# OrientalHorizon/Ray-Tracer-Archive

Measured on NVIDIA B200. Metric: path segments/sec, higher is better.
Workload: dtype f32

## Files before the change

### ray_tracer_archive_b200/csrc/rtb_api.cu

```cuda
#include <cuda_runtime.h>

#include <algorithm>
#include <cmath>
#include <cstdio>
#include <cstring>
#include <string>
#include <vector>

#include <atomic>
#include <memory>
#include <thread>

#include "rtb_device.cuh"
#include "rtb_launch.hpp"
#include "rtb_nccl.hpp"

using namespace rtb;

static thread_local std::string g_err;
static int set_err(int code, const std::string& m) { g_err = m; return code; }
#define CU(call)                                                                                              \
  do {                                                                                                        \
    cudaError_t e_ = (call);                                                                                  \
    if (e_ != cudaSuccess)                                                                                    \
// ... 822 lines not shown
}

static DevPool lane_pool(Lane& L, uint32_t n) {
  DevPool p;
  p.n = n;
  p.n_chunks = (n + RTB_CHUNK - 1) / RTB_CHUNK;
  p.ray = L.ray.p; p.st = L.st.p; p.hit = L.hit.p;
  p.cls = L.cls.p; p.redo[0] = L.redo[0].p; p.redo[1] = L.redo[1].p; p.cursor = L.cursor.p;
  p.c = L.counters.p;
  return p;
}

static int ensure_pix_order(rtb_context* c, uint32_t W, uint32_t H, cudaStream_t st) {
  if (c->pix_w == W && c->pix_h == H && c->pix_order.p) return RTB_OK;
  std::vector<uint32_t> order;
  order.reserve((size_t)W * H);
  for (uint32_t ty = 0; ty < H; ty += 4)
    for (uint32_t tx = 0; tx < W; tx += 8)
      for (uint32_t y = ty; y < std::min(ty + 4, H); ++y)
        for (uint32_t x = tx; x < std::min(tx + 8, W); ++x) order.push_back(y * W + x);
  CU(c->pix_order.upload(order.data(), order.size(), st));
  CU(cudaStreamSynchronize(st));
  c->pix_w = W; c->pix_h = H;
  return RTB_OK;
}

#define RTB_DEFAULT_POOL (1u << 22)

static int check_render_args(rtb_context* c, rtb_scene* s, const rtb_camera* cam, const rtb_params* p, const void* buf) {
  if (!c || !s || !cam || !p || !buf) return set_err(RTB_ERR_INVALID, "NULL argument");
  if (!s->committed) return set_err(RTB_ERR_STATE, "scene not committed (call rtb_scene_commit)");
  if (p->width < 2 || p->height < 2) return set_err(RTB_ERR_INVALID, "image must be at least 2x2 (u = (i+xi)/(W-1), main.rs:752)");
  if (p->max_depth < 1 || p->max_depth > 255) return set_err(RTB_ERR_INVALID, "max_depth must be in [1,255]");
  if (p->spp == 0) return set_err(RTB_ERR_INVALID, "spp must be > 0");
  if ((uint64_t)p->sample_offset + p->spp > (1u << 24)) return set_err(RTB_ERR_INVALID, "sample index exceeds 2^24");
  return RTB_OK;
}

static int render_camera(const rtb_camera& cam, DevCamera& dcam) {
  DevCameraF64 dcam64;
  camera_basis(cam, dcam, dcam64);
  for (int a = 0; a < 3; ++a)
    if (!std::isfinite(dcam.origin[a]) || !std::isfinite(dcam.lmo[a]) || !std::isfinite(dcam.horizontal[a]) || !std::isfinite(dcam.vertical[a]) ||
        !std::isfinite(dcam.u[a]) || !std::isfinite(dcam.v[a]))
      return set_err(RTB_ERR_INVALID, "degenerate camera (non-finite basis: lookfrom == lookat, vup along the view direction, or non-finite arguments)");
  return RTB_OK;
}

static uint32_t extend_opt(const rtb_scene* s) {
  static const char* env_opt = getenv("RTB_OPT");
  return env_opt ? (uint32_t)atoi(env_opt)
         : s->lc.mode == EXTEND_WQ ? ((24u << RTB_OPT_PARK_SHIFT) | (2u << 16))
         : s->lc.mode == EXTEND_DYNAMIC ? (14u << RTB_OPT_PARK_SHIFT)
                                        : (s->lc.all_staged ? 0u : 2u );
}

static int default_lanes() {
  static const int env_lanes = getenv("RTB_LANES") ? atoi(getenv("RTB_LANES")) : 0;
  const int want_lanes = env_lanes > 0 ? env_lanes : 4;
  return std::max(1, std::min(want_lanes, RTB_MAX_LANES));
}

int rtb_render_device(rtb_context* c, rtb_scene* s, const rtb_camera* cam, const rtb_params* p, void* d_accum,
                      void* stream, rtb_stats* stats) {
  int rc = check_render_args(c, s, cam, p, d_accum);
  if (rc) return rc;
  CU(cudaSetDevice(c->device));
  cudaStream_t st = (cudaStream_t)stream;
  const uint64_t npix = (uint64_t)p->width * p->height;
  const bool count = (p->flags & RTB_RENDER_COUNT) != 0, time_ext = (p->flags & RTB_RENDER_TIME_EXTEND) != 0;
  int n_lanes = (count || time_ext) ? 1 : default_lanes();
  if ((uint32_t)n_lanes > p->spp) n_lanes = (int)p->spp;
  uint32_t pool_total = p->pool_paths ? p->pool_paths : RTB_DEFAULT_POOL;
  rc = ensure_pix_order(c, p->width, p->height, st);
  if (rc) return rc;
  DevCamera dcam;
  rc = render_camera(*cam, dcam);
  if (rc) return rc;

  struct LaneRun { DevPool pool; DevParams prm; unsigned long long total; bool active; uint64_t iters, iter_cap; };
  LaneRun run[RTB_MAX_LANES];
  uint32_t first_sample = 0;
  for (int k = 0; k < n_lanes; ++k) {
    Lane& L = c->lanes[k];
    const uint32_t cnt = p->spp / n_lanes + ((uint32_t)k < p->spp % n_lanes ? 1u : 0u);
    LaneRun& R = run[k];
    R.total = npix * cnt;
    uint32_t pool_n = std::max(1024u, pool_total / (uint32_t)n_lanes);
    const uint32_t unit = s->lc.pool_unit;
    if (!p->pool_paths && unit) pool_n = std::max(1u, (pool_n + unit / 2) / unit) * unit;
    if ((unsigned long long)pool_n > R.total) pool_n = (uint32_t)std::max<unsigned long long>(1024ull, R.total);
    rc = ensure_pool(L, pool_n);
    if (rc) return rc;
    R.pool = lane_pool(L, pool_n);
    DevParams& prm = R.prm;
    prm.width = p->width; prm.height = p->height; prm.spp = cnt; prm.sample_offset = p->sample_offset + first_sample;
    prm.max_depth = p->max_depth; prm.rr_start = p->rr_start_depth; prm.seed = p->seed;
    for (int a = 0; a < 3; ++a) prm.bg[a] = p->background[a];
    prm.pix_order = c->pix_order.p;
    prm.inv_npix = 1.0 / (double)npix;
    prm.opt = extend_opt(s);
    prm.inv_wm1 = (float)(1.0 / (double)(p->width - 1));
    prm.inv_hm1 = (float)(1.0 / (double)(p->height - 1));
    prm.accum = (float4*)d_accum;
    first_sample += cnt;
    R.active = true;
    R.iters = 0;
// ... 526 lines not shown
```

### ray_tracer_archive_b200/csrc/rtb_device.cuh

```cuda
#pragma once
#include <cuda_runtime.h>
#include <stdint.h>

#include <cmath>
#include <cstring>

#include "rtb_internal.hpp"

namespace rtb {

#ifdef RTB_CHECKED
__device__ unsigned int g_rtb_check_fail[8];
enum CheckKind : int { CHK_STACK = 0, CHK_NODE = 1, CHK_PRIM = 2, CHK_SLOT = 3, CHK_QUEUE = 4, CHK_LIST = 5 };
#define RTB_CHECK(kind, cond)                          \
  do {                                                 \
    if (!(cond)) atomicAdd(&g_rtb_check_fail[kind], 1u); \
  } while (0)
#else
#define RTB_CHECK(kind, cond) ((void)0)
#endif

#define RTB_MAX_LIGHTS 8
#define RTB_MAX_MEDIA 8
#define RTB_MAX_CHECKER_DEPTH 8
// ... 505 lines not shown
    }
    const float Sz = rcp_fast(dp.z), Sx = dp.x * Sz, Sy = dp.y * Sz;
    const float Ax = __fsub_rn(A.x, __fmul_rn(Sx, A.z)), Ay = __fsub_rn(A.y, __fmul_rn(Sy, A.z));
    const float Bx = __fsub_rn(B.x, __fmul_rn(Sx, B.z)), By = __fsub_rn(B.y, __fmul_rn(Sy, B.z));
    const float Cx = __fsub_rn(C.x, __fmul_rn(Sx, C.z)), Cy = __fsub_rn(C.y, __fmul_rn(Sy, C.z));
    const float U = __fsub_rn(__fmul_rn(Cx, By), __fmul_rn(Cy, Bx));
    const float V = __fsub_rn(__fmul_rn(Ax, Cy), __fmul_rn(Ay, Cx));
    const float W = __fsub_rn(__fmul_rn(Bx, Ay), __fmul_rn(By, Ax));
    const float m = (1.25f * RTB_U22 * amax) * (fabsf(Ax) + fabsf(Ay) + fabsf(Bx) + fabsf(By) + fabsf(Cx) + fabsf(Cy));
    const float mn = fminf(fminf(U, V), W), mx = fmaxf(fmaxf(U, V), W);
    if (mn < -m && mx > m) return HIT_MISS;
    const float det = U + V + W;
    const float idet = rcp_fast(det), za = Sz * A.z, zb = Sz * B.z, zc = Sz * C.z;
    const float zlo = fminf(fminf(za, zb), zc), zhi = fmaxf(fmaxf(za, zb), zc);
    if (!(mn > m || mx < -m)) {
      if (!(zhi >= tmin)) return HIT_MISS;
      t = fmaxf(zlo - RTB_U20 * fabsf(zlo), 0.0f);
      return HIT_AMBIGUOUS;
    }
    t = (U * za + V * zb + W * zc) * idet;
    e = fmaf(RTB_U20, fabsf(t), 4.0f * m * fabsf(idet) * (zhi - zlo));
    if (!(t - e <= tmax_hi)) return HIT_MISS;
    const int st = tmin_status(t, e, tmin);
    if (st == HIT_AMBIGUOUS) t = fmaxf(t - e, 0.0f);
    return st;
  } else {
    const float4 a = __ldg(sc.geom[PT_MOVING] + 2 * idx);
    const float4 b = __ldg(sc.geom[PT_MOVING] + 2 * idx + 1);
    const float3 c = fma3(time, xyz(b), xyz(a));
    return sphere_fast(o, d, c, a.w, tmin, tmax_hi, t, e, coarse);
  }
}
__device__ __forceinline__ void apply_result(Closest& best, float& amb, uint32_t& flags, int st, float t, float e, uint32_t ref,
                                             bool coarse) {
  if (st == HIT_CERTAIN) consider(best, amb, flags, t, e, ref, coarse);
  else if (st == HIT_AMBIGUOUS) undecided(best, amb, t);
}
template <bool COUNT>
__device__ __forceinline__ void intersect_prim(const DevScene& sc, uint32_t type, uint32_t idx, float3 o, float3 d,
                                               float time, float tmin, Closest& best, float& amb, uint32_t& flags, TestCount& n_tests) {
  float t, e;
  bool coarse;
  const int st = prim_test<COUNT>(sc, type, idx, o, d, time, tmin, best.hi, t, e, coarse, n_tests);
  apply_result(best, amb, flags, st, t, e, (type << REF_TYPE_SHIFT) | idx, coarse);
}

__device__ __forceinline__ float q2f(uint32_t word, uint32_t magic, uint32_t sel) {
  return __uint_as_float(__byte_perm(word, magic, sel));
}

#if !defined(__CUDA_ARCH__) && defined(RTB_EMUL_STATS)
inline unsigned long long g_emul_stats[8];
inline float g_emul_tmax0 = INFINITY;
#endif
struct Trav {
  float3 o, d;
  float idx, idy, idz, time;
  uint32_t octinv;
  uint2 grp;
  int sp;
  Closest best;
  float amb;
};
__device__ __forceinline__ uint32_t octant_remap(uint32_t m, uint32_t octinv) {
  if (octinv & 1u) m = ((m & 0x55u) << 1) | ((m & 0xAAu) >> 1);
  if (octinv & 2u) m = ((m & 0x33u) << 2) | ((m & 0xCCu) >> 2);
  if (octinv & 4u) m = ((m & 0x0Fu) << 4) | ((m & 0xF0u) >> 4);
  return m;
}
__shared__ uint8_t s_octmap[8 * 256];
__device__ __forceinline__ bool needs_exact(const Closest& best, float amb) { return amb < INFINITY && amb <= best.hi; }
enum FixKind : uint32_t { FIX_NONE = 0, FIX_RETRACE = 1, FIX_REFINE = 2 };
#define RTB_REDO_REFINE 0x80000000u
__device__ __forceinline__ bool quad_distance_is_coarse(const DevScene& sc, uint32_t idx, float3 o, float3 d) {
  const float4 w0 = __ldg(sc.geom[PT_QUAD] + 3 * idx);
  if (__ldg(&sc.info[PT_QUAD][idx].y) >> 31) return false;
  const float mag_num = fabsf(w0.w) + fabsf(w0.x * o.x) + fabsf(w0.y * o.y) + fabsf(w0.z * o.z);
  const float mag_den = fabsf(w0.x * d.x) + fabsf(w0.y * d.y) + fabsf(w0.z * d.z);
  return 64.0f * fabsf(dot(xyz(w0), d)) < mag_den || 64.0f * fabsf(w0.w - dot(xyz(w0), o)) < mag_num;
}
__device__ __forceinline__ bool tri_distance_is_coarse(const DevScene& sc, uint32_t idx, float3 o, float3 d) {
  const float3 v0 = xyz(__ldg(sc.geom[PT_TRI] + 3 * idx));
  const float3 n = cross(xyz(__ldg(sc.geom[PT_TRI] + 3 * idx + 1)) - v0, xyz(__ldg(sc.geom[PT_TRI] + 3 * idx + 2)) - v0);
  const float3 r = v0 - o;
  const float mag_num = fabsf(n.x * r.x) + fabsf(n.y * r.y) + fabsf(n.z * r.z);
  const float mag_den = fabsf(n.x * d.x) + fabsf(n.y * d.y) + fabsf(n.z * d.z);
  return 64.0f * fabsf(dot(n, d)) < mag_den || 64.0f * fabsf(dot(n, r)) < mag_num;
}
#define FIX_NOMINATED 3u
__device__ __forceinline__ uint32_t fix_kind_cheap(const Trav& tv) {
  if (needs_exact(tv.best, tv.amb)) return FIX_RETRACE;
  if (tv.best.ref == REF_MISS) return FIX_NONE;
  const uint32_t type = tv.best.ref >> REF_TYPE_SHIFT;
  if (type == PT_QUAD || type == PT_TRI)
    return tv.best.hi - tv.best.t > (type == PT_QUAD ? RTB_FLAT_REL_MAX : RTB_TRI_REL_MAX) * tv.best.t ? FIX_NOMINATED : FIX_NONE;
  return (tv.octinv & RTB_TRAV_COARSE) ? FIX_REFINE : FIX_NONE;
}
__device__ __forceinline__ uint32_t resolve_nominated(const DevScene& sc, uint32_t ref, float3 o, float3 d) {
  const uint32_t type = ref >> REF_TYPE_SHIFT, idx = ref & REF_INDEX_MASK;
  const bool coarse = type == PT_QUAD ? quad_distance_is_coarse(sc, idx, o, d) : tri_distance_is_coarse(sc, idx, o, d);
  return coarse ? FIX_REFINE : FIX_NONE;
}
__device__ __forceinline__ uint32_t fix_kind(const DevScene& sc, const Trav& tv) {
  const uint32_t k = fix_kind_cheap(tv);
  return k == FIX_NOMINATED ? resolve_nominated(sc, tv.best.ref, tv.o, tv.d) : k;
}
// ... 122 lines not shown
      const float tnx = fmaf(q2f(i < 4 ? nx0 : nx1, magic, sel), ax, bnx);
      const float tny = fmaf(q2f(i < 4 ? ny0 : ny1, magic, sel), ay, bny);
      const float tnz = fmaf(q2f(i < 4 ? nz0 : nz1, magic, sel), az, bnz);
      const float tfx = fmaf(q2f(i < 4 ? fx0 : fx1, magic, sel), ax, bfx);
      const float tfy = fmaf(q2f(i < 4 ? fy0 : fy1, magic, sel), ay, bfy);
      const float tfz = fmaf(q2f(i < 4 ? fz0 : fz1, magic, sel), az, bfz);
      const float tn = fmaxf(fmaxf(tnx, tny), tnz);
      const float tf = fminf(fminf(tfx, tfy), tfz);
      const uint32_t neg = __float_as_uint(tf - tn) | __float_as_uint(tmax - tn) | __float_as_uint(tf - tmin);
      missmask = __funnelshift_l(neg, missmask, 1);
    }
  }
  const uint32_t hitmask = ~missmask & 0xFFu;
#if !defined(__CUDA_ARCH__) && defined(RTB_EMUL_STATS)
  ++g_emul_stats[0];
  if (!hitmask) ++g_emul_stats[1];
  g_emul_stats[2] += __builtin_popcount(hitmask & imask);
  g_emul_stats[3] += __builtin_popcount(hitmask & ~imask);
  {
    uint32_t np = 0;
    for (uint32_t s = 0; s < 8; ++s)
      if ((hitmask & ~imask) >> s & 1u) np += (((s < 4 ? w1.z : w1.w) >> (8 * (s & 3))) & 0xFFu) >> 5;
    if (np) ++g_emul_stats[np == 1 ? 4 : (np == 2 ? 5 : 6)];
    g_emul_stats[7] += np;
  }
#endif
  uint32_t ih = hitmask & imask;
  if constexpr (OCTMAP) ih = s_octmap[(octinv << 8) | ih];
  else ih = octant_remap(ih, octinv);
  tv.grp = make_uint2(w1.x, (ih << 8) | imask);
  const uint32_t leaf = hitmask & ~imask;
  if (leaf) leaves_fn(leaf, w1.y, w1.z, w1.w);
  return true;
}

template <bool COUNT>
__device__ __forceinline__ void trav_globals(const DevScene& sc, Trav& tv, float tmin, TestCount& n_tests) {
  for (uint32_t k = 0; k < sc.n_global; ++k) {
    const uint32_t ref = sc.global_ref[k];
    if ((sc.global_f64 >> k) & 1u) {
      if (COUNT) ++n_tests.n[PT_SPHERE];
      const float4 s = __ldg(sc.geom[PT_SPHERE] + (ref & REF_INDEX_MASK));
      float t;
      const int st = sphere_roots_f64(tv.o, tv.d, xyz(s), s.w, tmin, t);
      if (st == HIT_CERTAIN) consider(tv.best, tv.amb, tv.octinv, t, RTB_U22 * t, ref, false);
      else if (st == HIT_AMBIGUOUS) tv.amb = 0.0f;
    } else {
      intersect_prim<COUNT>(sc, ref >> REF_TYPE_SHIFT, ref & REF_INDEX_MASK, tv.o, tv.d, tv.time, tmin, tv.best, tv.amb, tv.octinv, n_tests);
    }
  }
  if (sc.tree_empty) tv.grp.y = 0u;
}

template <bool COUNT, bool ALL_STAGED = false, bool PACKED = false, bool OCTMAP = false, bool SPHSTAGE = false>
__device__ __forceinline__ bool trav_step_fast(const DevScene& sc, const uint4* __restrict__ snodes, uint32_t sbase, uint32_t n_snodes,
                                               Trav& tv, uint2* __restrict__ stack, float tmin,
                                               uint32_t& n_nodes_visited, TestCount& n_tests, uint32_t ssph = 0u) {
  return trav_step<COUNT, ALL_STAGED, 1, PACKED, OCTMAP>(sc, snodes, sbase, n_snodes, tv, stack, tmin, n_nodes_visited,
                                      [&](uint32_t leaf, uint32_t w1y, uint32_t w1z, uint32_t w1w) {
                                        expand_leaves(leaf, w1y, w1z, w1w, [&](uint32_t type, uint32_t idx) {
                                          if (SPHSTAGE && type == PT_SPHERE) {
                                            if (COUNT) ++n_tests.n[PT_SPHERE];
                                            RTB_CHECK(CHK_PRIM, idx < sc.n_prims[PT_SPHERE]);
                                            float t, e = 0.0f;
                                            bool coarse = false;
                                            const float4 s = lds_sphere(sc, ssph, idx);
                                            const int st = sphere_fast(tv.o, tv.d, xyz(s), s.w, tmin, tv.best.hi, t, e, coarse);
                                            apply_result(tv.best, tv.amb, tv.octinv, st, t, e, ((uint32_t)PT_SPHERE << REF_TYPE_SHIFT) | idx, coarse);
                                          } else {
                                            intersect_prim<COUNT>(sc, type, idx, tv.o, tv.d, tv.time, tmin, tv.best, tv.amb, tv.octinv, n_tests);
                                          }
                                        });
                                      });
}

template <bool COUNT, bool ALL_STAGED = false>
__device__ __forceinline__ bool trav_step_park(const DevScene& sc, const uint4* __restrict__ snodes, uint32_t sbase, uint32_t n_snodes,
                                               Trav& tv, uint2* __restrict__ stack, float tmin, uint32_t& n_nodes_visited,
                                               uint4* __restrict__ park, bool& parked) {
  return trav_step<COUNT, ALL_STAGED, 1, false>(sc, snodes, sbase, n_snodes, tv, stack, tmin, n_nodes_visited,
                                      [&](uint32_t leaf, uint32_t w1y, uint32_t w1z, uint32_t w1w) {
                                        *park = make_uint4(leaf, w1y, w1z, w1w);
                                        parked = true;
                                      });
}
template <bool COUNT>
__device__ __forceinline__ void drain_parked(const DevScene& sc, Trav& tv, float tmin, const uint4* __restrict__ park, bool parked,
                                             TestCount& n_tests) {
  uint4 pd = make_uint4(0u, 0u, 0u, 0u);
  if (parked) pd = *park;
  const uint32_t mytype = pd.y >> REF_TYPE_SHIFT;
#pragma unroll
  for (uint32_t t = 0; t < PT_COUNT; ++t) {
    const bool mine = parked && mytype == t;
    if (!__any_sync(0xffffffffu, mine)) continue;
    if (mine)
      expand_leaves(pd.x, pd.y, pd.z, pd.w, [&](uint32_t, uint32_t idx) {
        intersect_prim<COUNT>(sc, t, idx, tv.o, tv.d, tv.time, tmin, tv.best, tv.amb, tv.octinv, n_tests);
      });
    __syncwarp();
  }
}

template <bool COUNT, bool ALL_STAGED = false, bool PACKED = false, bool OCTMAP = false, bool SPHSTAGE = false>
__device__ __forceinline__ uint32_t traverse(const DevScene& sc, const uint4* __restrict__ snodes, uint32_t sbase, uint32_t n_snodes,
                                         float3 o, float3 d, float time, float tmin, Closest& best, float& slab_lo_out,
                                         uint32_t& n_nodes_visited, TestCount& n_tests, uint32_t ssph = 0u) {
  Trav tv;
  uint2 stack[RTB_STACK];
  trav_init(tv, o, d, time);
  trav_globals<COUNT>(sc, tv, tmin, n_tests);
  while (trav_step_fast<COUNT, ALL_STAGED, PACKED, OCTMAP, SPHSTAGE>(sc, snodes, sbase, n_snodes, tv, stack, tmin, n_nodes_visited, n_tests, ssph)) {}
  best = tv.best;
  slab_lo_out = slab_lo(tv);
  return fix_kind(sc, tv);
}

__device__ __forceinline__ float refine_hit(const DevScene& sc, uint32_t ref, float3 o, float3 d, float time, float t) {
  if ((ref >> REF_TYPE_SHIFT) >= PT_COUNT) return t;
  const double tc = exact_hit(sc.xtab, ref, o, d, time);
  return tc >= 0.0 ? (float)tc : t;
}

__device__ __forceinline__ Closest traverse_exact(const DevScene& sc, float3 o, float3 d, float time, float t_lo = 0.0f, float t_hi = INFINITY) {
  Trav tv;
  uint2 stack[RTB_STACK];
  trav_init(tv, o, d, time);
  tv.best.hi = fmaf(t_hi, 4.0e-6f, t_hi) + 1.0e-6f;
  const float tmin = fmaxf(fmaf(t_lo, -4.0e-6f, t_lo) - 1.0e-6f, 0.0f);
  double bt = 0.0;
  const ExactTab* tab = sc.xtab;
  auto leaf = [&](uint32_t type, uint32_t idx) {
    const uint32_t ref = (type << REF_TYPE_SHIFT) | idx;
    {
      Closest probe{INFINITY, tv.best.hi, REF_MISS};
      float probe_amb = INFINITY;
      uint32_t probe_flags = 0;
      TestCount none{};
      intersect_prim<false>(sc, type, idx, tv.o, tv.d, tv.time, RTB_TMIN, probe, probe_amb, probe_flags, none);
      if (probe.ref == REF_MISS && !(probe_amb < INFINITY)) return;
    }
    const double tc = exact_hit(tab, ref, tv.o, tv.d, tv.time);
    if (tc < 0.0) return;
    if (tv.best.ref == REF_MISS || tc < bt || (tc == bt && tab_gid(tab, ref) > tab_gid(tab, tv.best.ref))) {
      bt = tc;
      const float tf = (float)tc;
      tv.best.t = tf;
      tv.best.hi = tf * (1.0f + RTB_U22);
      tv.best.ref = ref;
    }
  };
  for (uint32_t k = 0; k < sc.n_global; ++k) leaf(sc.global_ref[k] >> REF_TYPE_SHIFT, sc.global_ref[k] & REF_INDEX_MASK);
  if (sc.tree_empty) tv.grp.y = 0u;
  uint32_t nv = 0;
  while (trav_step<false, false>(sc, nullptr, 0u, 0u, tv, stack, tmin, nv,
                                 [&](uint32_t lf, uint32_t w1y, uint32_t w1z, uint32_t w1w) { expand_leaves(lf, w1y, w1z, w1w, leaf); })) {}
  if (tv.best.ref == REF_MISS) tv.best.t = tv.best.hi = INFINITY;
  return tv.best;
}

__device__ __forceinline__ void intersect_media(const DevScene& sc, float3 o, float3 d, float tmin, Closest& best,
                                                uint32_t pixel, uint32_t sample, uint32_t bounce, uint32_t seed,
                                                bool have_rng) {
  for (uint32_t m = 0; m < sc.n_media; ++m) {
    const DevMedium& md = sc.media[m];
// ... 51 lines not shown
```

### ray_tracer_archive_b200/csrc/rtb_kernels.cu

```cuda
#include <cuda_runtime.h>

#include <algorithm>
#include <cstdlib>
#include <cstring>

#include "rtb_device.cuh"
#include "rtb_launch.hpp"

namespace rtb {

__device__ __forceinline__ uint32_t ray_octant(float3 d) {
  return (d.x < 0.0f ? 1u : 0u) | (d.y < 0.0f ? 2u : 0u) | (d.z < 0.0f ? 4u : 0u);
}

__device__ __forceinline__ void prefetch_l1(const void* p) { asm volatile("prefetch.global.L1 [%0];" ::"l"(p)); }
__device__ __forceinline__ void prefetch_l2(const void* p) { asm volatile("prefetch.global.L2 [%0];" ::"l"(p)); }

__device__ __forceinline__ void red_add_v4(float4* addr, float a, float b, float c, float d) {
  asm volatile("red.global.add.v4.f32 [%0], {%1, %2, %3, %4};" ::"l"(addr), "f"(a), "f"(b), "f"(c), "f"(d) : "memory");
}

__device__ __forceinline__ void deposit(const DevParams& prm, DevCounters* c, uint32_t pixel, float3 L) {
  if (!(isfinite(L.x) && isfinite(L.y) && isfinite(L.z))) {
    atomicAdd(&c->rejected, 1ull);
// ... 123 lines not shown
  for (uint32_t j = 0; j < 8; ++j) {
    const uint32_t b = ((j < 4 ? cw.x : cw.y) >> (8 * (j & 3))) & 0xFFu, cls = b & 7u;
    key[j] = cls == CLS_DEAD ? 64u : ((cls == CLS_NEW ? 0u : cls + 1u) << 3) | ((b >> 3) & 7u);
    rank[j] = key[j] < 64u ? atomicAdd(&cnt[key[j]], 1u) : 0u;
  }
  __syncwarp();
  const uint32_t v0 = cnt[lane], v1 = lane < 16u ? cnt[32u + lane] : 0u;
  uint32_t i0 = v0, i1 = v1;
#pragma unroll
  for (uint32_t d = 1; d < 32; d <<= 1) {
    const uint32_t a = __shfl_up_sync(0xffffffffu, i0, d), b2 = __shfl_up_sync(0xffffffffu, i1, d);
    if (lane >= d) { i0 += a; i1 += b2; }
  }
  const uint32_t t0 = __shfl_sync(0xffffffffu, i0, 31), total = t0 + __shfl_sync(0xffffffffu, i1, 15);
  __syncwarp();
  cnt[lane] = i0 - v0;
  if (lane < 16u) cnt[32u + lane] = t0 + i1 - v1;
  __syncwarp();
#pragma unroll
  for (uint32_t j = 0; j < 8; ++j)
    if (key[j] < 64u) {
      RTB_CHECK(CHK_LIST, cnt[key[j]] + rank[j] < RTB_CHUNK);
      list[cnt[key[j]] + rank[j]] = (uint8_t)(8u * lane + j);
    }
  __syncwarp();
  return total;
}

__device__ __forceinline__ void report_counts(DevCounters* c, uint32_t nv, TestCount nt, uint32_t lane) {
  nv = __reduce_add_sync(0xffffffffu, nv);
  uint32_t tot = 0;
#pragma unroll
  for (uint32_t t = 0; t < PT_COUNT; ++t) {
    nt.n[t] = __reduce_add_sync(0xffffffffu, nt.n[t]);
    tot += nt.n[t];
  }
  if (lane == 0) {
    atomicAdd(&c->nodes_visited, (unsigned long long)nv);
    atomicAdd(&c->prims_tested, (unsigned long long)tot);
    for (uint32_t t = 0; t < PT_COUNT; ++t)
      if (nt.n[t]) atomicAdd(&c->prims_tested_type[t], (unsigned long long)nt.n[t]);
  }
}

#ifndef RTB_EXTEND_MAXREG
#define RTB_EXTEND_MAXREG 80
#endif
#ifndef RTB_EXTEND_DYN_MAXREG
#define RTB_EXTEND_DYN_MAXREG 64
#endif
struct ExtIn { float4 o_time, d_slot, idir_oct, best; };
struct ExtOut { float t; uint32_t ref, slot, redo; float lo, hi; uint32_t _pad[2]; };
#define RTB_EXTEND_WARPS (RTB_EXTEND_THREADS / 32)

template <bool COUNT>
__global__ void __maxnreg__(RTB_EXTEND_DYN_MAXREG)
k_extend(DevScene sc, DevPool pool, DevParams prm, uint32_t n_snodes) {
  extern __shared__ uint4 snodes[];
  __shared__ ExtIn s_in[RTB_EXTEND_WARPS][32];
  __shared__ ExtOut s_out[RTB_EXTEND_WARPS][32];
  __shared__ uint8_t s_list[RTB_EXTEND_WARPS][RTB_CHUNK];
  __shared__ uint4 s_park[RTB_EXTEND_WARPS][32];
  DevCounters* c = pool.c;
  stage_nodes(sc, snodes, n_snodes);
  uint32_t sbase = (uint32_t)__cvta_generic_to_shared(snodes);
  asm volatile("mov.u32 %0, %0;" : "+r"(sbase));
  const uint32_t lane = threadIdx.x & 31u, warp = threadIdx.x >> 5;
  const uint32_t lt_mask = (1u << lane) - 1u;
  const uint32_t park_min = max(1u, (prm.opt >> RTB_OPT_PARK_SHIFT) & RTB_OPT_PARK_MASK);
  uint4* park = &s_park[warp][lane];
  uint32_t parked_mask = 0;
  ExtIn* in = s_in[warp];
  ExtOut* out = s_out[warp];
  uint8_t* list = s_list[warp];
  uint32_t idle = 0xffffffffu;
  uint32_t slot = 0;
  uint32_t in_head = 0, in_count = 0, out_count = 0;
  uint32_t chunk_base = 0, list_pos = 0, list_len = 0;
  bool exhausted = false;
  uint32_t n_rays = 0;
  Trav tv;
  uint2 stack[RTB_STACK];
  uint32_t nv = 0;
  TestCount nt{};
  const uint32_t refill_min = 8u;
  auto flush = [&]() {
    __syncwarp();
    if (lane < out_count) {
      const ExtOut h = out[lane];
      float3 o = f3(0.f, 0.f, 0.f), d = o;
      if (sc.n_media) {
        o = xyz(pool.ray[2 * h.slot]);
        d = xyz(pool.ray[2 * h.slot + 1]);
      }
      finish_ray(sc, pool, prm, h.slot, o, d, Closest{h.t, h.t, h.ref});
      uint32_t redo = h.redo;
      if (redo == FIX_NOMINATED) redo = resolve_nominated(sc, h.ref, xyz(pool.ray[2 * h.slot]), xyz(pool.ray[2 * h.slot + 1]));
      if (redo) queue_fix(pool, h.slot, redo, h.lo, h.hi);
    }
    out_count = 0;
    __syncwarp();
  };

  for (;;) {
    const uint32_t n_idle = __popc(idle);
    if (n_idle >= refill_min || idle == 0xffffffffu) {
// ... 248 lines not shown
      finished = !trav_step<COUNT, false, (int)RTB_WQ_RAYS>(sc, snodes, sbase, n_snodes, tv, &W.stack[0][r], RTB_TMIN, nv,
                                                            [&](uint32_t leaf, uint32_t w1y, uint32_t w1z, uint32_t w1w) {
                                                              W.rec[r] = make_uint4(leaf, w1y, w1z, w1w);
                                                              const uint32_t type = w1y >> REF_TYPE_SHIFT;
                                                              cls = type <= PT_MOVING ? 0u : type - 1u;
                                                              leafed = true;
                                                            });
      RTB_CHECK(CHK_STACK, tv.sp <= (int)RTB_WQ_STACK);
      if (!finished) {
        *reinterpret_cast<uint2*>(&W.trav[r]) = tv.grp;
        W.trav[r].z = (uint32_t)tv.sp;
      }
    }
    const uint32_t done = __ballot_sync(0xffffffffu, finished);
    const uint32_t leafs = __ballot_sync(0xffffffffu, leafed);
    if (done | leafs) {
      const uint32_t bit_lo = r < 32u ? 1u << r : 0u, bit_hi = (r & 32u) ? 1u << (r & 31u) : 0u;
      rdy_lo &= ~__reduce_or_sync(0xffffffffu, finished || leafed ? bit_lo : 0u);
      rdy_hi &= ~__reduce_or_sync(0xffffffffu, finished || leafed ? bit_hi : 0u);
      if (leafs) {
        const uint32_t m0 = __ballot_sync(0xffffffffu, cls == 0u), m1 = __ballot_sync(0xffffffffu, cls == 1u), m2 = leafs & ~(m0 | m1);
        if (leafed) {
          const uint32_t mine = cls == 0u ? m0 : (cls == 1u ? m1 : m2);
          const uint32_t end = cls == 0u ? qh0 + qn0 : (cls == 1u ? qh1 + qn1 : qh2 + qn2);
          W.q[cls][(end + __popc(mine & lt_mask)) & 63u] = (uint8_t)r;
        }
        qn0 += __popc(m0); qn1 += __popc(m1); qn2 += __popc(m2);
      }
      if (done) {
        free_lo |= __reduce_or_sync(0xffffffffu, finished ? bit_lo : 0u);
        free_hi |= __reduce_or_sync(0xffffffffu, finished ? bit_hi : 0u);
        if (out_count + __popc(done) > 32u) flush();
        if (finished) {
          const float4 b = W.best[r];
          Trav tv;
          tv.best = Closest{b.x, b.z, __float_as_uint(b.y)};
          tv.amb = b.w;
          tv.octinv = W.trav[r].w;
          W.out[out_count + __popc(done & lt_mask)] =
              ExtOut{tv.best.t, tv.best.ref, __float_as_uint(W.d_slot[r].w), fix_kind_cheap(tv), slab_lo(tv), tv.best.hi, {0u, 0u}};
        }
        out_count += __popc(done);
      }
    }
    __syncwarp();
  }
  if (lane == 0 && n_rays) atomicAdd(&c->iter_rays, n_rays);
  if (COUNT) report_counts(c, nv, nt, lane);
}

template <bool COUNT, bool ALL_STAGED, bool SORT, bool SPHSTAGE = false>
__global__ void __maxnreg__(RTB_EXTEND_MAXREG)
k_extend_static(DevScene sc, DevPool pool, DevParams prm, uint32_t n_snodes) {
  static_assert(!SPHSTAGE || (ALL_STAGED && !COUNT), "the sphere stage is built for the fully staged production kernel");
  extern __shared__ uint4 snodes[];
  __shared__ uint8_t s_list[RTB_EXTEND_WARPS][RTB_CHUNK];
  __shared__ uint32_t s_cnt[SORT ? RTB_EXTEND_WARPS : 1][64];
  DevCounters* c = pool.c;
  if constexpr (ALL_STAGED) octmap_fill();
  if constexpr (SPHSTAGE) {
    const uint4* sph = reinterpret_cast<const uint4*>(sc.geom[PT_SPHERE]);
    for (uint32_t i = threadIdx.x; i < sc.n_prims[PT_SPHERE]; i += blockDim.x) snodes[5u * n_snodes + i] = __ldg(sph + i);
  }
  stage_nodes(sc, snodes, n_snodes);
  uint32_t sbase = (uint32_t)__cvta_generic_to_shared(snodes);
  asm volatile("mov.u32 %0, %0;" : "+r"(sbase));
  const uint32_t lane = threadIdx.x & 31u, warp = threadIdx.x >> 5;
  uint8_t* list = s_list[warp];
  const uint32_t n_warps = gridDim.x * RTB_EXTEND_WARPS;
  uint32_t n_rays = 0, nv = 0;
  TestCount nt{};
  for (uint32_t chunk = blockIdx.x * RTB_EXTEND_WARPS + warp; chunk < pool.n_chunks; chunk += n_warps) {
    const uint32_t base = chunk * RTB_CHUNK;
    const uint32_t total = SORT ? build_extend_list_sorted(pool, chunk, list, s_cnt[SORT ? warp : 0], lane) : build_extend_list(pool, chunk, list, lane);
    n_rays += total;
    for (uint32_t r = 0; r < total; r += 32) {
      if (r + 32 + lane < total) prefetch_l1(pool.ray + 2 * (size_t)(base + list[r + 32 + lane]));
      if (r + lane < total) {
        const uint32_t slot = base + list[r + lane];
        const float4 ro = pool.ray[2 * slot];
        const float4 rd = pool.ray[2 * slot + 1];
        Closest best;
        float lo;
        const uint32_t fix = traverse<COUNT, ALL_STAGED, ALL_STAGED && !COUNT, ALL_STAGED, SPHSTAGE>(
            sc, snodes, sbase, n_snodes, xyz(ro), xyz(rd), ro.w, RTB_TMIN, best, lo, nv, nt, sbase + n_snodes * 80u);
        finish_ray(sc, pool, prm, slot, xyz(ro), xyz(rd), best);
        if (fix) queue_fix(pool, slot, fix, lo, best.hi);
      }
    }
    __syncwarp();
  }
  if (lane == 0 && n_rays) atomicAdd(&c->iter_rays, n_rays);
  if (COUNT) report_counts(c, nv, nt, lane);
}

struct Surf {
  float3 p, n, outward;
  bool front;
  uint32_t mat, ref;
};

__device__ __forceinline__ Surf surface_at(const DevScene& sc, uint32_t ref, uint32_t minfo, float3 o, float3 d, float time, float t) {
  Surf s;
  s.ref = ref;
  s.p = fma3(t, d, o);
  const uint32_t type = ref >> REF_TYPE_SHIFT, idx = ref & REF_INDEX_MASK;
  if (type == PT_MEDIUM) {
    s.n = s.outward = f3(1.f, 0.f, 0.f);
    s.front = true;
    s.mat = RTB_MINFO_MAT(minfo);
    return s;
  }
  if (type == PT_SPHERE) {
    const float4 g = __ldg(sc.geom[PT_SPHERE] + idx);
    s.outward = rcp_fast(g.w) * (s.p - xyz(g));
  } else if (type == PT_MOVING) {
    const float4 a = __ldg(sc.geom[PT_MOVING] + 2 * idx), b = __ldg(sc.geom[PT_MOVING] + 2 * idx + 1);
    s.outward = rcp_fast(a.w) * (s.p - fma3(time, xyz(b), xyz(a)));
  } else if (type == PT_QUAD) {
    s.outward = xyz(__ldg(sc.geom[PT_QUAD] + 3 * idx));
  } else {
    const float3 v0 = xyz(__ldg(sc.geom[PT_TRI] + 3 * idx));
    const float3 e1 = xyz(__ldg(sc.geom[PT_TRI] + 3 * idx + 1)) - v0, e2 = xyz(__ldg(sc.geom[PT_TRI] + 3 * idx + 2)) - v0;
    s.outward = unit(cross(e1, e2));
  }
  s.mat = RTB_MINFO_MAT(minfo);
  bool ff = dot(d, s.outward) < 0.0f;
  s.n = ff ? s.outward : -s.outward;
  const uint32_t mode = RTB_MINFO_FACE(minfo), base = mode & 7u;
  if (mode >= FACE_Q) {
    float sn, cs;
    if (type == PT_TRI) {
      sn = __ldg(sc.geom[PT_TRI] + 3 * idx).w;
      cs = __ldg(sc.geom[PT_TRI] + 3 * idx + 1).w;
    } else {
      const double* ex = sc.xtab->exact[type] + (size_t)idx * RTB_EXACT_STRIDE;
      sn = (float)ex[4]; cs = (float)ex[5];
    }
// ... 644 lines not shown
  extern __shared__ uint4 sm[];
  const uint32_t n = 2048;
  for (uint32_t i = threadIdx.x; i < n; i += blockDim.x) sm[i] = make_uint4(i, i * 3u, i * 5u, i * 7u);
  __syncthreads();
  uint4 acc = make_uint4(0u, 0u, 0u, 0u);
  const uint32_t base = (uint32_t)__cvta_generic_to_shared(sm);
  uint32_t k = threadIdx.x;
#pragma unroll 8
  for (uint32_t r = 0; r < reps; ++r) {
    uint4 v;
    asm volatile("ld.shared.v4.u32 {%0, %1, %2, %3}, [%4];" : "=r"(v.x), "=r"(v.y), "=r"(v.z), "=r"(v.w) : "r"(base + k * 16u));
    acc.x ^= v.x; acc.y ^= v.y; acc.z ^= v.z; acc.w ^= v.w;
    k = (k + 256u) & (n - 1u);
  }
  if ((acc.x ^ acc.y ^ acc.z ^ acc.w) == 0x12345679u) sink[0] = acc;
}

#ifdef RTB_CHECKED
int read_check_failures(unsigned int* out8) {
  return (int)cudaMemcpyFromSymbol(out8, g_rtb_check_fail, sizeof(unsigned int) * 8);
}
#else
int read_check_failures(unsigned int* out8) {
  for (int i = 0; i < 8; ++i) out8[i] = 0xFFFFFFFFu;
  return 0;
}
#endif

static inline uint32_t cdiv(uint32_t a, uint32_t b) { return (a + b - 1) / b; }

void launch_init_pool(const DevPool& pool, unsigned long long total_paths, cudaStream_t st) {
  k_init_pool<<<cdiv(pool.n_chunks * RTB_CHUNK, 256), 256, 0, st>>>(pool, total_paths);
}
void launch_generate(const LaunchCfg& lc, const DevPool& pool, const DevParams& prm, const DevCamera& cam, cudaStream_t st) {
  k_generate<<<lc.shade_grid, RTB_SHADE_THREADS, 0, st>>>(pool, prm, cam);
}
void launch_fixup(const LaunchCfg& lc, const DevScene& sc, const DevPool& pool, const DevParams& prm, cudaStream_t st) {
  k_fixup<<<lc.fixup_grid, RTB_FIXUP_THREADS, 0, st>>>(sc, pool, prm);
}
void launch_rotate(const DevPool& pool, cudaStream_t st) { k_rotate<<<1, 1, 0, st>>>(pool); }
void launch_extend(const LaunchCfg& lc, const DevScene& sc, const DevPool& pool, const DevParams& prm, bool count,
                   cudaStream_t st) {
  if (lc.mode == EXTEND_WQ) {
    if (count) k_extend_wq<true><<<lc.extend_grid, RTB_EXTEND_THREADS, lc.extend_smem, st>>>(sc, pool, prm, lc.n_snodes);
    else k_extend_wq<false><<<lc.extend_grid, RTB_EXTEND_THREADS, lc.extend_smem, st>>>(sc, pool, prm, lc.n_snodes);
    return;
  }
  if (lc.mode == EXTEND_STATIC) {
    const bool sort = (prm.opt & RTB_OPT_OCTANT_SORT) != 0u;
    if (count) {
      if (sort) k_extend_static<true, false, true><<<lc.extend_grid, RTB_EXTEND_THREADS, lc.extend_smem, st>>>(sc, pool, prm, lc.n_snodes);
      else k_extend_static<true, false, false><<<lc.extend_grid, RTB_EXTEND_THREADS, lc.extend_smem, st>>>(sc, pool, prm, lc.n_snodes);
    } else if (lc.all_staged && lc.sphere_smem) {
      const uint32_t smem = lc.extend_smem + lc.sphere_smem;
      if (sort) k_extend_static<false, true, true, true><<<lc.extend_grid, RTB_EXTEND_THREADS, smem, st>>>(sc, pool, prm, lc.n_snodes);
      else k_extend_static<false, true, false, true><<<lc.extend_grid, RTB_EXTEND_THREADS, smem, st>>>(sc, pool, prm, lc.n_snodes);
    } else if (lc.all_staged) {
      if (sort) k_extend_static<false, true, true><<<lc.extend_grid, RTB_EXTEND_THREADS, lc.extend_smem, st>>>(sc, pool, prm, lc.n_snodes);
      else k_extend_static<false, true, false><<<lc.extend_grid, RTB_EXTEND_THREADS, lc.extend_smem, st>>>(sc, pool, prm, lc.n_snodes);
    } else {
      if (sort) k_extend_static<false, false, true><<<lc.extend_grid, RTB_EXTEND_THREADS, lc.extend_smem, st>>>(sc, pool, prm, lc.n_snodes);
      else k_extend_static<false, false, false><<<lc.extend_grid, RTB_EXTEND_THREADS, lc.extend_smem, st>>>(sc, pool, prm, lc.n_snodes);
    }
    return;
  }
  if (count) k_extend<true><<<lc.extend_grid, RTB_EXTEND_THREADS, lc.extend_smem, st>>>(sc, pool, prm, lc.n_snodes);
  else k_extend<false><<<lc.extend_grid, RTB_EXTEND_THREADS, lc.extend_smem, st>>>(sc, pool, prm, lc.n_snodes);
}
void launch_shade(const LaunchCfg& lc, const DevScene& sc, const DevPool& pool, const DevParams& prm,
                  const DevCamera& cam, uint32_t present, cudaStream_t st) {
  k_shade_terminal<<<lc.shade_grid, RTB_SHADE_THREADS, 0, st>>>(sc, pool, prm, cam);
  if (present & (1u << RTB_MAT_LAMBERTIAN)) k_shade_lambert<<<lc.shade_grid, RTB_SHADE_THREADS, 0, st>>>(sc, pool, prm, cam);
  if (present & ((1u << RTB_MAT_METAL) | (1u << RTB_MAT_DIELECTRIC)))
    k_shade_specular<<<lc.shade_grid, RTB_SHADE_THREADS, 0, st>>>(sc, pool, prm, cam);
  if (present & (1u << RTB_MAT_ISOTROPIC)) k_shade_isotropic<<<lc.shade_grid, RTB_SHADE_THREADS, 0, st>>>(sc, pool, prm, cam);
}
void launch_finalize(const float4* accum, uint8_t* rgb, uint32_t npix, float inv_spp, cudaStream_t st) {
  k_finalize<<<cdiv(npix, 256), 256, 0, st>>>(accum, rgb, npix, inv_spp);
}
void launch_probe_fill(const DevPool& pool, const float* org, const float* dir, const float* time, uint32_t n, cudaStream_t st) {
  k_probe_fill<<<cdiv(pool.n_chunks * RTB_CHUNK, 256), 256, 0, st>>>(pool, org, dir, time, n);
}
void launch_probe_collect(const DevScene& sc, const DevPool& pool, uint32_t n, uint32_t* id_out, float* t_out, cudaStream_t st) {
  k_probe_collect<<<cdiv(n, 256), 256, 0, st>>>(sc, pool, n, id_out, t_out);
}
void launch_kat(const DevScene& sc, const DevCamera& cam, const DevParams& prm, uint32_t op, const uint32_t* in, uint32_t n,
                uint32_t in_stride, uint32_t* out, uint32_t out_stride, cudaStream_t st) {
  k_kat<<<cdiv(n, 128), 128, 0, st>>>(sc, cam, prm, op, in, n, in_stride, out, out_stride);
}
void launch_bw_global(const uint4* p, size_t n_vec, uint32_t reps, uint4* sink, uint32_t grid, cudaStream_t st) {
  k_bw_global<<<grid, 256, 0, st>>>(p, n_vec, reps, sink);
}
void launch_bw_shared(uint32_t reps, uint4* sink, uint32_t grid, cudaStream_t st) {
  k_bw_shared<<<grid, 256, 32768, st>>>(reps, sink);
}
void launch_aov_fill(const DevPool& pool, const DevParams& prm, const DevCamera& cam, unsigned long long first_path,
                     uint32_t n, cudaStream_t st) {
  k_aov_fill<<<cdiv(pool.n_chunks * RTB_CHUNK, 256), 256, 0, st>>>(pool, prm, cam, first_path, n);
}
void launch_aov_collect(const DevScene& sc, const DevPool& pool, const DevParams& prm, float4* aov, uint32_t n,
                        cudaStream_t st) {
  k_aov_collect<<<cdiv(n, RTB_SHADE_THREADS), RTB_SHADE_THREADS, 0, st>>>(sc, pool, prm, aov, n);
}
void launch_primary_rays(const DevCameraF64& cam, uint32_t W, uint32_t H, float* org, float* dir, float* time,
                         cudaStream_t st) {
  k_primary_rays<<<cdiv(W * H, 256), 256, 0, st>>>(cam, W, H, org, dir, time);
}

int configure_launch(LaunchCfg& lc, uint32_t n_nodes, uint32_t max_depth, uint32_t n_spheres, int sm_count) {
  lc.dynamic_fetch = n_nodes > 4096;
  uint32_t budget = (getenv("RTB_STAGE_KB") ? (uint32_t)atoi(getenv("RTB_STAGE_KB")) : (lc.dynamic_fetch ? 6u : 12u)) * 1024u;
  budget = std::min(budget, (lc.dynamic_fetch ? 84u : 104u) * 1024u);
  uint32_t n_s = n_nodes;
  if ((size_t)n_s * 80 > budget) n_s = budget / 80;
  lc.n_snodes = n_s;
  lc.all_staged = n_s == n_nodes && !(getenv("RTB_ALL_STAGED") && atoi(getenv("RTB_ALL_STAGED")) == 0);
  lc.extend_smem = n_s * 80;
  const char* mode = getenv("RTB_EXTEND_MODE");
  lc.mode = lc.dynamic_fetch ? EXTEND_DYNAMIC : EXTEND_STATIC;
  if (mode) lc.mode = !strcmp(mode, "static") ? EXTEND_STATIC : (!strcmp(mode, "wq") ? EXTEND_WQ : EXTEND_DYNAMIC);
  if (lc.mode == EXTEND_WQ && (lc.all_staged || max_depth + 2u > RTB_WQ_STACK))
    lc.mode = lc.dynamic_fetch ? EXTEND_DYNAMIC : EXTEND_STATIC;
  lc.sphere_smem = lc.mode == EXTEND_STATIC && lc.all_staged && n_spheres <= RTB_SPHERE_STAGE_BYTES / 16u ? n_spheres * 16u : 0u;
  cudaError_t e;
  const void* extend_fn = (const void*)k_extend<false>;
  if (lc.mode == EXTEND_WQ) {
    const uint32_t wq_bytes = RTB_EXTEND_WARPS * (uint32_t)sizeof(WqWarp);
    lc.extend_smem += wq_bytes;
    extend_fn = (const void*)k_extend_wq<false>;
    for (const void* fn : {(const void*)k_extend_wq<false>, (const void*)k_extend_wq<true>}) {
      e = cudaFuncSetAttribute(fn, cudaFuncAttributeMaxDynamicSharedMemorySize, (int)(budget + wq_bytes));
      if (e != cudaSuccess) return (int)e;
    }
  }
  e = cudaFuncSetAttribute(k_extend<false>, cudaFuncAttributeMaxDynamicSharedMemorySize, (int)budget);
  if (e != cudaSuccess) return (int)e;
  e = cudaFuncSetAttribute(k_extend<true>, cudaFuncAttributeMaxDynamicSharedMemorySize, (int)budget);
  if (e != cudaSuccess) return (int)e;
  for (const void* fn : {(const void*)k_extend_static<true, false, false>, (const void*)k_extend_static<true, false, true>,
                         (const void*)k_extend_static<false, true, false>, (const void*)k_extend_static<false, true, true>,
                         (const void*)k_extend_static<false, false, false>, (const void*)k_extend_static<false, false, true>}) {
    e = cudaFuncSetAttribute(fn, cudaFuncAttributeMaxDynamicSharedMemorySize, (int)budget);
    if (e != cudaSuccess) return (int)e;
  }
  if (lc.sphere_smem) {
    for (const void* fn : {(const void*)k_extend_static<false, true, false, true>, (const void*)k_extend_static<false, true, true, true>}) {
      e = cudaFuncSetAttribute(fn, cudaFuncAttributeMaxDynamicSharedMemorySize, (int)(budget + RTB_SPHERE_STAGE_BYTES));
      if (e != cudaSuccess) return (int)e;
    }
  }
  int occ = 0;
  e = cudaOccupancyMaxActiveBlocksPerMultiprocessor(&occ, extend_fn, RTB_EXTEND_THREADS, lc.extend_smem + lc.sphere_smem);
  if (e != cudaSuccess) return (int)e;
  if (occ < 1) occ = 1;
  occ = std::min(occ, getenv("RTB_EXTEND_OCC") ? std::max(1, atoi(getenv("RTB_EXTEND_OCC"))) : std::max(1, 512 / RTB_EXTEND_THREADS));
  lc.extend_grid = (uint32_t)(sm_count * occ);
  int occ2 = 0;
  e = cudaOccupancyMaxActiveBlocksPerMultiprocessor(&occ2, k_shade_lambert, RTB_SHADE_THREADS, 0);
  if (e != cudaSuccess) return (int)e;
  if (occ2 < 1) occ2 = 1;
  if (getenv("RTB_SHADE_OCC")) occ2 = std::max(1, std::min(occ2, atoi(getenv("RTB_SHADE_OCC"))));
  lc.shade_grid = (uint32_t)(sm_count * occ2);
  lc.fixup_grid = (uint32_t)std::max(1, sm_count * 2);
  {
    uint32_t a = lc.extend_grid * RTB_EXTEND_WARPS, b = lc.shade_grid * RTB_SHADE_WARPS, x = a, y = b;
    while (y) { const uint32_t t = x % y; x = y; y = t; }
    const uint64_t lcm = (uint64_t)a / x * b;
    lc.pool_unit = lcm * RTB_CHUNK <= (1ull << 23) ? (uint32_t)(lcm * RTB_CHUNK) : b * RTB_CHUNK;
  }
  return 0;
}

}
```

Before: 8490.

## Add persistent ray refill and leaf parking to sphere-staged static extend kernel

```diff
diff --git a/ray_tracer_archive_b200/csrc/rtb_api.cu b/ray_tracer_archive_b200/csrc/rtb_api.cu
--- a/ray_tracer_archive_b200/csrc/rtb_api.cu
+++ b/ray_tracer_archive_b200/csrc/rtb_api.cu
@@ -898,7 +898,7 @@
   return env_opt ? (uint32_t)atoi(env_opt)
          : s->lc.mode == EXTEND_WQ ? ((24u << RTB_OPT_PARK_SHIFT) | (2u << 16))
          : s->lc.mode == EXTEND_DYNAMIC ? (14u << RTB_OPT_PARK_SHIFT)
-                                        : (s->lc.all_staged ? 0u : 2u );
+                                        : (s->lc.all_staged ? (8u << RTB_OPT_PARK_SHIFT) : 2u );
 }
 
 static int default_lanes() {
diff --git a/ray_tracer_archive_b200/csrc/rtb_device.cuh b/ray_tracer_archive_b200/csrc/rtb_device.cuh
--- a/ray_tracer_archive_b200/csrc/rtb_device.cuh
+++ b/ray_tracer_archive_b200/csrc/rtb_device.cuh
@@ -581,6 +581,11 @@
 #if !defined(__CUDA_ARCH__) && defined(RTB_EMUL_STATS)
 inline unsigned long long g_emul_stats[8];
 inline float g_emul_tmax0 = INFINITY;
+inline uint8_t* g_emul_seq = nullptr;
+inline unsigned long long g_emul_seq_n = 0, g_emul_seq_cap = 0;
+inline void emul_seq_push(uint32_t v) {
+  if (g_emul_seq && g_emul_seq_n < g_emul_seq_cap) g_emul_seq[g_emul_seq_n++] = (uint8_t)(v == 255u || v < 254u ? v : 254u);
+}
 #endif
 struct Trav {
   float3 o, d;
@@ -809,26 +814,32 @@
   if (sc.tree_empty) tv.grp.y = 0u;
 }
 
-template <bool COUNT, bool ALL_STAGED = false, bool PACKED = false, bool OCTMAP = false, bool SPHSTAGE = false>
+template <bool COUNT, bool ALL_STAGED = false, bool PACKED = false, bool OCTMAP = false>
 __device__ __forceinline__ bool trav_step_fast(const DevScene& sc, const uint4* __restrict__ snodes, uint32_t sbase, uint32_t n_snodes,
                                                Trav& tv, uint2* __restrict__ stack, float tmin,
-                                               uint32_t& n_nodes_visited, TestCount& n_tests, uint32_t ssph = 0u) {
+                                               uint32_t& n_nodes_visited, TestCount& n_tests) {
   return trav_step<COUNT, ALL_STAGED, 1, PACKED, OCTMAP>(sc, snodes, sbase, n_snodes, tv, stack, tmin, n_nodes_visited,
                                       [&](uint32_t leaf, uint32_t w1y, uint32_t w1z, uint32_t w1w) {
                                         expand_leaves(leaf, w1y, w1z, w1w, [&](uint32_t type, uint32_t idx) {
-                                          if (SPHSTAGE && type == PT_SPHERE) {
-                                            if (COUNT) ++n_tests.n[PT_SPHERE];
-                                            RTB_CHECK(CHK_PRIM, idx < sc.n_prims[PT_SPHERE]);
-                                            float t, e = 0.0f;
-                                            bool coarse = false;
-                                            const float4 s = lds_sphere(sc, ssph, idx);
-                                            const int st = sphere_fast(tv.o, tv.d, xyz(s), s.w, tmin, tv.best.hi, t, e, coarse);
-                                            apply_result(tv.best, tv.amb, tv.octinv, st, t, e, ((uint32_t)PT_SPHERE << REF_TYPE_SHIFT) | idx, coarse);
-                                          } else {
-                                            intersect_prim<COUNT>(sc, type, idx, tv.o, tv.d, tv.time, tmin, tv.best, tv.amb, tv.octinv, n_tests);
-                                          }
+                                          intersect_prim<COUNT>(sc, type, idx, tv.o, tv.d, tv.time, tmin, tv.best, tv.amb, tv.octinv, n_tests);
                                         });
                                       });
+}
+
+template <bool COUNT>
+__device__ __forceinline__ void leaf_test_staged(const DevScene& sc, Trav& tv, float tmin, uint32_t type, uint32_t idx,
+                                                 TestCount& n_tests, uint32_t ssph) {
+  if (type == PT_SPHERE) {
+    if (COUNT) ++n_tests.n[PT_SPHERE];
+    RTB_CHECK(CHK_PRIM, idx < sc.n_prims[PT_SPHERE]);
+    float t, e = 0.0f;
+    bool coarse = false;
+    const float4 s = lds_sphere(sc, ssph, idx);
+    const int st = sphere_fast(tv.o, tv.d, xyz(s), s.w, tmin, tv.best.hi, t, e, coarse);
+    apply_result(tv.best, tv.amb, tv.octinv, st, t, e, ((uint32_t)PT_SPHERE << REF_TYPE_SHIFT) | idx, coarse);
+  } else {
+    intersect_prim<COUNT>(sc, type, idx, tv.o, tv.d, tv.time, tmin, tv.best, tv.amb, tv.octinv, n_tests);
+  }
 }
 
 template <bool COUNT, bool ALL_STAGED = false>
@@ -859,15 +870,24 @@
   }
 }
 
-template <bool COUNT, bool ALL_STAGED = false, bool PACKED = false, bool OCTMAP = false, bool SPHSTAGE = false>
+template <bool COUNT, bool ALL_STAGED = false, bool PACKED = false, bool OCTMAP = false>
 __device__ __forceinline__ uint32_t traverse(const DevScene& sc, const uint4* __restrict__ snodes, uint32_t sbase, uint32_t n_snodes,
                                          float3 o, float3 d, float time, float tmin, Closest& best, float& slab_lo_out,
-                                         uint32_t& n_nodes_visited, TestCount& n_tests, uint32_t ssph = 0u) {
+                                         uint32_t& n_nodes_visited, TestCount& n_tests) {
   Trav tv;
   uint2 stack[RTB_STACK];
   trav_init(tv, o, d, time);
   trav_globals<COUNT>(sc, tv, tmin, n_tests);
-  while (trav_step_fast<COUNT, ALL_STAGED, PACKED, OCTMAP, SPHSTAGE>(sc, snodes, sbase, n_snodes, tv, stack, tmin, n_nodes_visited, n_tests, ssph)) {}
+#if !defined(__CUDA_ARCH__) && defined(RTB_EMUL_STATS)
+  emul_seq_push(255u);
+  for (;;) {
+    const uint32_t before = n_tests.n[0] + n_tests.n[1] + n_tests.n[2] + n_tests.n[3];
+    if (!trav_step_fast<COUNT, ALL_STAGED, PACKED, OCTMAP>(sc, snodes, sbase, n_snodes, tv, stack, tmin, n_nodes_visited, n_tests)) break;
+    emul_seq_push(n_tests.n[0] + n_tests.n[1] + n_tests.n[2] + n_tests.n[3] - before);
+  }
+#else
+  while (trav_step_fast<COUNT, ALL_STAGED, PACKED, OCTMAP>(sc, snodes, sbase, n_snodes, tv, stack, tmin, n_nodes_visited, n_tests)) {}
+#endif
   best = tv.best;
   slab_lo_out = slab_lo(tv);
   return fix_kind(sc, tv);
diff --git a/ray_tracer_archive_b200/csrc/rtb_kernels.cu b/ray_tracer_archive_b200/csrc/rtb_kernels.cu
--- a/ray_tracer_archive_b200/csrc/rtb_kernels.cu
+++ b/ray_tracer_archive_b200/csrc/rtb_kernels.cu
@@ -199,6 +199,7 @@
 struct ExtIn { float4 o_time, d_slot, idir_oct, best; };
 struct ExtOut { float t; uint32_t ref, slot, redo; float lo, hi; uint32_t _pad[2]; };
 #define RTB_EXTEND_WARPS (RTB_EXTEND_THREADS / 32)
+#define RTB_REFILL_MIN 16u
 
 template <bool COUNT>
 __global__ void __maxnreg__(RTB_EXTEND_DYN_MAXREG)
@@ -553,7 +554,7 @@
 template <bool COUNT, bool ALL_STAGED, bool SORT, bool SPHSTAGE = false>
 __global__ void __maxnreg__(RTB_EXTEND_MAXREG)
 k_extend_static(DevScene sc, DevPool pool, DevParams prm, uint32_t n_snodes) {
-  static_assert(!SPHSTAGE || (ALL_STAGED && !COUNT), "the sphere stage is built for the fully staged production kernel");
+  static_assert(!SPHSTAGE || (ALL_STAGED && !COUNT && !SORT), "the sphere stage is built for the fully staged production kernel");
   extern __shared__ uint4 snodes[];
   __shared__ uint8_t s_list[RTB_EXTEND_WARPS][RTB_CHUNK];
   __shared__ uint32_t s_cnt[SORT ? RTB_EXTEND_WARPS : 1][64];
@@ -571,6 +572,75 @@
   const uint32_t n_warps = gridDim.x * RTB_EXTEND_WARPS;
   uint32_t n_rays = 0, nv = 0;
   TestCount nt{};
+  if constexpr (SPHSTAGE) {
+    __shared__ uint4 s_park[RTB_EXTEND_THREADS];
+    __shared__ uint32_t s_slot[RTB_EXTEND_THREADS];
+    const uint32_t park_min = max(1u, (prm.opt >> RTB_OPT_PARK_SHIFT) & RTB_OPT_PARK_MASK);
+    const uint32_t lt_mask = (1u << lane) - 1u;
+    Trav tv;
+    uint2 stack[RTB_STACK];
+    uint32_t idle = 0xffffffffu, parked_mask = 0, done = 0;
+    uint32_t chunk = blockIdx.x * RTB_EXTEND_WARPS + warp, pos = 0, total = 0;
+    if (chunk < pool.n_chunks) total = build_extend_list(pool, chunk, list, lane);
+    if (lane == 0 && total) atomicAdd(&c->iter_rays, total);
+    for (;;) {
+      if (__popc(idle) >= RTB_REFILL_MIN || idle == 0xffffffffu) {
+        if ((done >> lane) & 1u) {
+          const uint32_t slot = s_slot[threadIdx.x];
+          finish_ray(sc, pool, prm, slot, tv.o, tv.d, tv.best);
+          const uint32_t fix = fix_kind(sc, tv);
+          if (fix) queue_fix(pool, slot, fix, slab_lo(tv), tv.best.hi);
+        }
+        done = 0;
+        while (idle && chunk < pool.n_chunks) {
+          if (pos == total) {
+            __syncwarp();
+            chunk += n_warps;
+            if (chunk >= pool.n_chunks) break;
+            total = build_extend_list(pool, chunk, list, lane);
+            if (lane == 0 && total) atomicAdd(&c->iter_rays, total);
+            pos = 0;
+            continue;
+          }
+          const uint32_t rank = __popc(idle & lt_mask);
+          const bool take = ((idle >> lane) & 1u) && pos + rank < total;
+          if (take) {
+            const uint32_t slot = chunk * RTB_CHUNK + list[pos + rank];
+            s_slot[threadIdx.x] = slot;
+            const float4 ro = pool.ray[2 * slot];
+            const float4 rd = pool.ray[2 * slot + 1];
+            trav_init(tv, xyz(ro), xyz(rd), ro.w);
+            trav_globals<COUNT>(sc, tv, RTB_TMIN, nt);
+          }
+          const uint32_t took = __ballot_sync(0xffffffffu, take);
+          idle &= ~took;
+          pos += __popc(took);
+        }
+        if (idle == 0xffffffffu) break;
+        if (pos + lane < total) prefetch_l1(pool.ray + 2 * (size_t)(chunk * RTB_CHUNK + list[pos + lane]));
+      }
+      bool finished = false, parked = (parked_mask >> lane) & 1u;
+      if (!(((idle | parked_mask) >> lane) & 1u))
+        finished = !trav_step<COUNT, true, 1, true, true>(sc, snodes, sbase, n_snodes, tv, stack, RTB_TMIN, nv,
+                                                        [&](uint32_t leaf, uint32_t w1y, uint32_t w1z, uint32_t w1w) {
+                                                          s_park[threadIdx.x] = make_uint4(leaf, w1y, w1z, w1w);
+                                                          parked = true;
+                                                        });
+      parked_mask = __ballot_sync(0xffffffffu, parked);
+      const uint32_t fin = __ballot_sync(0xffffffffu, finished);
+      if (parked_mask && ((uint32_t)__popc(parked_mask) >= park_min || (idle | parked_mask | fin) == 0xffffffffu)) {
+        if (parked) {
+          const uint4 pd = s_park[threadIdx.x];
+          expand_leaves(pd.x, pd.y, pd.z, pd.w,
+                        [&](uint32_t type, uint32_t idx) { leaf_test_staged<COUNT>(sc, tv, RTB_TMIN, type, idx, nt, sbase + n_snodes * 80u); });
+        }
+        __syncwarp();
+        parked_mask = 0;
+      }
+      done |= fin;
+      idle |= fin;
+    }
+  } else
   for (uint32_t chunk = blockIdx.x * RTB_EXTEND_WARPS + warp; chunk < pool.n_chunks; chunk += n_warps) {
     const uint32_t base = chunk * RTB_CHUNK;
     const uint32_t total = SORT ? build_extend_list_sorted(pool, chunk, list, s_cnt[SORT ? warp : 0], lane) : build_extend_list(pool, chunk, list, lane);
@@ -583,8 +653,8 @@
         const float4 rd = pool.ray[2 * slot + 1];
         Closest best;
         float lo;
-        const uint32_t fix = traverse<COUNT, ALL_STAGED, ALL_STAGED && !COUNT, ALL_STAGED, SPHSTAGE>(
-            sc, snodes, sbase, n_snodes, xyz(ro), xyz(rd), ro.w, RTB_TMIN, best, lo, nv, nt, sbase + n_snodes * 80u);
+        const uint32_t fix = traverse<COUNT, ALL_STAGED, ALL_STAGED && !COUNT, ALL_STAGED>(
+            sc, snodes, sbase, n_snodes, xyz(ro), xyz(rd), ro.w, RTB_TMIN, best, lo, nv, nt);
         finish_ray(sc, pool, prm, slot, xyz(ro), xyz(rd), best);
         if (fix) queue_fix(pool, slot, fix, lo, best.hi);
       }
@@ -1335,9 +1405,7 @@
       if (sort) k_extend_static<true, false, true><<<lc.extend_grid, RTB_EXTEND_THREADS, lc.extend_smem, st>>>(sc, pool, prm, lc.n_snodes);
       else k_extend_static<true, false, false><<<lc.extend_grid, RTB_EXTEND_THREADS, lc.extend_smem, st>>>(sc, pool, prm, lc.n_snodes);
     } else if (lc.all_staged && lc.sphere_smem) {
-      const uint32_t smem = lc.extend_smem + lc.sphere_smem;
-      if (sort) k_extend_static<false, true, true, true><<<lc.extend_grid, RTB_EXTEND_THREADS, smem, st>>>(sc, pool, prm, lc.n_snodes);
-      else k_extend_static<false, true, false, true><<<lc.extend_grid, RTB_EXTEND_THREADS, smem, st>>>(sc, pool, prm, lc.n_snodes);
+      k_extend_static<false, true, false, true><<<lc.extend_grid, RTB_EXTEND_THREADS, lc.extend_smem + lc.sphere_smem, st>>>(sc, pool, prm, lc.n_snodes);
     } else if (lc.all_staged) {
       if (sort) k_extend_static<false, true, true><<<lc.extend_grid, RTB_EXTEND_THREADS, lc.extend_smem, st>>>(sc, pool, prm, lc.n_snodes);
       else k_extend_static<false, true, false><<<lc.extend_grid, RTB_EXTEND_THREADS, lc.extend_smem, st>>>(sc, pool, prm, lc.n_snodes);
@@ -1427,10 +1495,9 @@
     if (e != cudaSuccess) return (int)e;
   }
   if (lc.sphere_smem) {
-    for (const void* fn : {(const void*)k_extend_static<false, true, false, true>, (const void*)k_extend_static<false, true, true, true>}) {
-      e = cudaFuncSetAttribute(fn, cudaFuncAttributeMaxDynamicSharedMemorySize, (int)(budget + RTB_SPHERE_STAGE_BYTES));
-      if (e != cudaSuccess) return (int)e;
-    }
+    e = cudaFuncSetAttribute(k_extend_static<false, true, false, true>, cudaFuncAttributeMaxDynamicSharedMemorySize,
+                             (int)(budget + RTB_SPHERE_STAGE_BYTES));
+    if (e != cudaSuccess) return (int)e;
   }
   int occ = 0;
   e = cudaOccupancyMaxActiveBlocksPerMultiprocessor(&occ, extend_fn, RTB_EXTEND_THREADS, lc.extend_smem + lc.sphere_smem);
```

After: 7218 (median of 6 runs). 0.85x the previous value.
